# ColumbiaDVMM/ColumbiaImageSearch

Hardware: AMD Instinct MI355X
Metric: queries/sec @ recall@10 on 10M LOPQ index (higher is better)
Workload: dtype f64

## Files before the change

columbiaimagesearch_amd/_lib.py:

```python
import ctypes
import os
from ctypes import POINTER, c_char_p, c_double, c_float, c_int, c_int32, c_int64, c_uint8, c_uint16, c_uint32, c_void_p

import numpy as np

CIS_F32, CIS_F64 = 4, 8
CIS_OK, CIS_EINVAL, CIS_EHIP, CIS_ENOMEM, CIS_EUNSUPPORTED, CIS_ENODEVICE = 0, -1, -2, -3, -4, -5

_HERE = os.path.dirname(os.path.abspath(__file__))
LIB_PATH = os.environ.get("CIS_LIB_PATH") or os.path.join(_HERE, "lib", "libcis_hip.so")


class cis_hit(ctypes.Structure):
    _fields_ = [("dist", c_double), ("visit_rank", c_uint32), ("pos", c_uint32), ("id", c_int64),
                ("cell", c_int32), ("reserved", c_int32)]


HIT_DTYPE = np.dtype([("dist", "<f8"), ("visit_rank", "<u4"), ("pos", "<u4"), ("id", "<i8"),
                      ("cell", "<i4"), ("reserved", "<i4")])
assert HIT_DTYPE.itemsize == ctypes.sizeof(cis_hit) == 32


class HipError(RuntimeError):
    """A HIP runtime call inside libcis_hip.so failed (or no gfx950 device is visible)."""


_PROTOS = {
    "cis_version": (c_int, []),
    "cis_last_error": (c_char_p, []),
    "cis_alloc_stats": (c_int, [POINTER(c_int64), POINTER(c_int64)]),
    "cis_device_count": (c_int, []),
    "cis_set_device": (c_int, [c_int]),
    "cis_selftest": (c_int, [POINTER(c_int)]),
    "cis_model_create": (c_int, [POINTER(c_void_p), c_int, c_int, c_int, c_int, c_int, c_int, c_void_p, c_void_p,
                                 c_void_p, c_void_p, c_void_p, c_void_p, c_int, c_int]),
    "cis_model_destroy": (None, [c_void_p]),
    "cis_apply_pca": (c_int, [c_void_p, c_void_p, c_int, c_int64, c_void_p]),
    "cis_encode": (c_int, [c_void_p, c_void_p, c_int, c_int64, c_void_p, c_void_p]),
    "cis_encode_dev": (c_int, [c_void_p, c_void_p, c_int, c_int64, c_void_p, c_void_p, c_void_p]),
    "cis_predict_coarse": (c_int, [c_void_p, c_void_p, c_int, c_int64, c_void_p]),
    "cis_project": (c_int, [c_void_p, c_void_p, c_int, c_int64, c_void_p, c_void_p]),
    "cis_predict_fine": (c_int, [c_void_p, c_void_p, c_int, c_int64, c_void_p, c_void_p]),
    "cis_subquantizer_distances": (c_int, [c_void_p, c_void_p, c_int, c_int64, c_void_p, c_void_p]),
    "cis_reconstruct": (c_int, [c_void_p, c_void_p, c_void_p, c_int64, c_void_p]),
    "cis_predict_cluster": (c_int, [c_void_p, c_int, c_void_p, c_int, c_int64, c_int, c_int, c_void_p]),
    "cis_multisequence": (c_int, [c_void_p, c_int, c_void_p, c_void_p, c_int, c_int64, c_int, c_int, c_int, c_void_p, c_void_p,
                                  POINTER(c_int)]),
    "cis_index_create": (c_int, [POINTER(c_void_p), c_void_p]),
    "cis_index_destroy": (None, [c_void_p]),
    "cis_index_create_view": (c_int, [POINTER(c_void_p), c_void_p]),
    "cis_index_insert_counters": (c_int, [c_void_p, c_void_p]),
    "cis_index_set_shard": (c_int, [c_void_p, c_int, c_int, c_void_p]),
    "cis_index_cell_counts": (c_int, [c_void_p, c_void_p]),
    "cis_index_add_remote_counts": (c_int, [c_void_p, c_void_p]),
    "cis_index_add": (c_int, [c_void_p, c_void_p, c_void_p, c_void_p, c_int64, c_int, POINTER(c_int64)]),
    "cis_index_size": (c_int64, [c_void_p]),
    "cis_index_add_dev": (c_int, [c_void_p, c_void_p, c_void_p, c_void_p, c_int64, c_int, POINTER(c_int64), POINTER(c_int64),
                                  c_void_p, c_void_p]),
    "cis_l2_normalize_dev": (c_int, [c_void_p, c_int, c_int64, c_int, c_void_p]),
    "cis_index_cell_counts_dev": (c_int, [c_void_p, c_void_p, c_void_p]),
    "cis_index_add_remote_counts_dev": (c_int, [c_void_p, c_void_p, c_void_p]),
    "cis_index_route_pack_dev": (c_int, [c_void_p, c_void_p, c_void_p, c_void_p, c_int64, c_void_p, c_void_p, c_void_p]),
    "cis_index_add_records_dev": (c_int, [c_void_p, c_void_p, c_int64, c_int, POINTER(c_int64), POINTER(c_int64), c_void_p,
                                          c_void_p]),
    "cis_index_get_cell": (c_int, [c_void_p, c_int, c_int, c_int64, c_void_p, c_void_p, POINTER(c_int64)]),
    "cis_index_get_codes": (c_int, [c_void_p, c_void_p, c_void_p, c_int64, c_void_p]),
    "cis_index_search": (c_int, [c_void_p, c_void_p, c_int, c_int, c_int64, c_int, c_void_p, c_void_p, c_void_p,
                                 c_void_p, c_void_p, c_void_p]),
    "cis_index_search_async": (c_int, [c_void_p, c_void_p, c_int, c_int, c_int64, c_int, c_void_p, c_void_p, c_void_p,
                                       c_void_p, c_void_p, c_void_p]),
    "cis_index_search_wait": (c_int, [c_void_p]),
    "cis_host_alloc": (c_int, [POINTER(c_void_p), ctypes.c_size_t]),
    "cis_host_free": (None, [c_void_p]),
    "cis_index_search_dev": (c_int, [c_void_p, c_void_p, c_int, c_int, c_int64, c_int, c_void_p, c_void_p, c_void_p,
                                     c_void_p, c_void_p, c_void_p, c_void_p]),
    "cis_index_search_partial_dev": (c_int, [c_void_p, c_void_p, c_int, c_int, c_int64, c_int, c_void_p, c_void_p,
                                             c_void_p]),
    "cis_index_query_owners_dev": (c_int, [c_void_p, c_void_p, c_int, c_int, c_int64, c_void_p, c_void_p, c_void_p]),
    "cis_routed_merge_tables_dev": (c_int, [c_void_p, c_int, c_int, c_void_p, c_void_p, c_int, c_void_p, c_void_p, c_void_p]),
    "cis_route_queries_dev": (c_int, [c_void_p, c_int, c_int, c_void_p, c_int, c_int, c_void_p, c_void_p, c_void_p, c_void_p, c_void_p]),
    "cis_index_search_partial_packed_dev": (c_int, [c_void_p, c_void_p, c_int, c_int, c_int64, c_int, c_void_p, c_void_p,
                                                    c_void_p, c_void_p, c_void_p, c_void_p]),
    "cis_merge_hits_dev": (c_int, [c_void_p, c_int, c_int, c_int, c_void_p, c_void_p, c_void_p, c_void_p, c_void_p,
                                   c_void_p]),
    "cis_merge_packed_dev": (c_int, [c_void_p, c_int, c_int64, c_void_p, c_void_p, c_int, c_int, c_void_p, c_void_p,
                                     c_void_p, c_void_p, c_void_p, c_void_p]),
# ... 153 lines not shown
```

columbiaimagesearch_amd/csrc/lopq_search.hip:

```cpp
#include "lopq_batch.h"

template <typename CT>
__global__ __launch_bounds__(256) void k_tables(const CT* __restrict__ X , const CT* __restrict__ Cs,
                                                const double* __restrict__ Rt, const double* __restrict__ mus,
                                                const double* __restrict__ subs, const TabDesc* __restrict__ tabs,
                                                int V, int h, int w, int nf, int K, int D,
                                                double* __restrict__ T , PwProg prog_w,
                                                double* __restrict__ px_out ,
                                                const int* __restrict__ tab_order, int first) {
    extern __shared__ __attribute__((aligned(16))) char smem[];
    double* v = reinterpret_cast<double*>(smem);
    double* px = v + h;
    const int tab = tab_order ? tab_order[first + blockIdx.x] : first + (int)blockIdx.x;
    const TabDesc td = tabs[tab];
    const int s = td.split, c = td.cluster;
    const CT* x = X + (int64_t)td.q * D + s * h;
    const CT* Cc = Cs + ((int64_t)s * V + c) * h;
    const double* mu = mus + ((int64_t)s * V + c) * h;
    const double* R = Rt + ((int64_t)s * V + c) * h * h;
    for (int k = threadIdx.x; k < h; k += blockDim.x) {
        const CT res = x[k] - Cc[k];
        v[k] = (double)res - mu[k];
    }
    __syncthreads();
// ... 174 lines not shown
                for (int u = 0; u < CH; ++u) ra[u] = Ra[(int64_t)(s0 + u) * 4 * h];
#pragma unroll
                for (int u = 0; u < CH; ++u) rb[u] = vb[4 * (s0 + u)];
#pragma unroll
                for (int u = 0; u < CH; ++u) acc = __builtin_amdgcn_mfma_f64_16x16x4f64(ra[u], rb[u], acc, 0, 0, 0);
            }
            if (mine) {
                double* o = so + t * opitch + it * 16 + kq;
#pragma unroll
                for (int r = 0; r < 4; ++r) o[4 * r] = acc[r];
            }
        }
    }
    __syncthreads();
    for (int e = tid; e < nt * h; e += 256) {
        const int tt = e / h, i = e - tt * h;
        const double a = so[tt * opitch + i];
        px_out[(int64_t)s_tab[tt] * h + i] = a;
        if (px32_out) px32_out[(int64_t)s_tab[tt] * h + i] = (float)a;
    }
}

template <typename CT>
static void launch_tables(int64_t n_tabs, size_t tab_lds, hipStream_t st, const CT* X, const CT* Cs, const double* Rt,
                          const double* mus, const double* subs, const TabDesc* tabs, const int* tab_order, int V, int h, int w,
                          int nf, int K, int D, double* T, PwProg prog_w, double* px_out, const int64_t* d_totals = nullptr,
                          float* px32_out = nullptr) {
    constexpr int TB = 8;
    if (px_out && h <= 256 && h % 16 == 0 && !getenv("CIS_TABLES_UNGROUPED") && !getenv("CIS_TABLES_VALU")) {
        const size_t lds = (size_t)16 * (h + 4 + h + 2) * sizeof(double);
        if (h % 64 == 0)
            hipLaunchKernelGGL((k_tables_group_mfma<CT, 16>), dim3((unsigned)ceil_div(n_tabs, 16)), dim3(256), lds, st, X, Cs, Rt, mus, tabs,
                               tab_order, (int)n_tabs, V, h, D, px_out, d_totals, px32_out);
        else
            hipLaunchKernelGGL((k_tables_group_mfma<CT, 4>), dim3((unsigned)ceil_div(n_tabs, 16)), dim3(256), lds, st, X, Cs, Rt, mus, tabs,
                               tab_order, (int)n_tabs, V, h, D, px_out, d_totals, px32_out);
    } else if (px_out && h <= 256 && 256 / h >= 1 && !getenv("CIS_TABLES_UNGROUPED")) {
        const size_t lds = (size_t)(TB * h + TB * h) * sizeof(double);
        hipLaunchKernelGGL((k_tables_group<CT, TB>), dim3((unsigned)ceil_div(n_tabs, TB)), dim3(256), lds, st, X, Cs, Rt, mus, tabs,
                           tab_order, (int)n_tabs, V, h, D, px_out, d_totals, px32_out);
    } else {
        hipLaunchKernelGGL(k_tables<CT>, dim3((unsigned)n_tabs), dim3(256), tab_lds, st, X, Cs, Rt, mus, subs, tabs, V, h, w, nf, K, D, T,
                           prog_w, px_out, (const int*)nullptr, 0);
    }
}

template <int W, int TPB = 64>
__global__ __launch_bounds__(256) void k_tables_from_px(const double* __restrict__ px ,
                                                        TabDesc* __restrict__ tabs, int n_tabs,
                                                        const double* __restrict__ subs, int h, int nf, int K,
                                                        double* __restrict__ T ,
                                                        float* __restrict__ T32 ,
                                                        const int64_t* __restrict__ d_totals ) {
    __shared__ double sf[TPB][W];
    __shared__ int ssplit[TPB];
    const int j = blockIdx.y, z = blockIdx.z, k = threadIdx.x;
    const int t0 = blockIdx.x * TPB;
    if (d_totals) {
        n_tabs = (int)d_totals[1];
        if (t0 >= n_tabs) return;
    }
    const int nt = (n_tabs - t0 < TPB) ? (n_tabs - t0) : TPB;
    for (int e = threadIdx.x; e < nt * W; e += 256) {
        const int t = e / W, i = e - t * W;
        sf[t][i] = px[(int64_t)(t0 + t) * h + j * W + i];
    }
    if (threadIdx.x < nt) ssplit[threadIdx.x] = tabs[t0 + threadIdx.x].split;
    __syncthreads();
    const bool on = k < K;
    double sc[W];
    const double* src = subs + ((int64_t)(z * nf + j) * K + (on ? k : 0)) * W;
#pragma unroll
    for (int i = 0; i < W; ++i) sc[i] = src[i];
    for (int t = 0; t < nt; ++t) {
        if (ssplit[t] != z) continue;
        const double* f = sf[t];
        auto elem = [&](int i) -> double { const double df = f[i] - sc[i]; return df * df; };
        const double v = pw_leaf<double>(elem, 0, W);
        const float v32 = (float)v;
        if (on) {
            __builtin_nontemporal_store(v, &T[((int64_t)(t0 + t) * nf + j) * K + k]);
            if (T32) T32[((int64_t)(t0 + t) * nf + j) * K + k] = v32;
        }
        uint32_t b = on ? __float_as_uint(v32) : 0u, dummy = 0u;
        wave_minmax_step<1>(dummy, b); wave_minmax_step<2>(dummy, b); wave_minmax_step<4>(dummy, b);
        wave_minmax_step<8>(dummy, b); wave_minmax_step<16>(dummy, b); wave_minmax_step<32>(dummy, b);
        if ((threadIdx.x & 63) == 0) atomicMax(reinterpret_cast<unsigned int*>(&tabs[t0 + t].pad), b);
    }
}

__global__ void k_tables_f32(const double* __restrict__ T, int64_t n, int nf, int K, float* __restrict__ T32, TabDesc* __restrict__ tabs) {
    const int64_t e = (int64_t)blockIdx.x * blockDim.x + threadIdx.x;
    if (e >= n) return;
    const float v = (float)T[e];
    T32[e] = v;
    atomicMax(reinterpret_cast<unsigned int*>(&tabs[e / ((int64_t)nf * K)].pad), __float_as_uint(v));
}

template <int N, int NT, bool PAY>
__device__ __forceinline__ void block_bitonic(uint64_t* ka, uint64_t* kb, int64_t* pay) {
    for (int k = 2; k <= N; k <<= 1) {
        for (int j = k >> 1; j > 0; j >>= 1) {
            for (int t = threadIdx.x; t < N / 2; t += NT) {
                const int i = ((t / j) * 2 * j) + (t % j);
                const int p = i + j;
                const bool asc = ((i & k) == 0);
                const uint64_t a0 = ka[i], b0 = kb[i], a1 = ka[p], b1 = kb[p];
                const bool gt = (a0 > a1) || (a0 == a1 && b0 > b1);
                if (gt == asc) {
                    ka[i] = a1; kb[i] = b1; ka[p] = a0; kb[p] = b0;
                    if (PAY) { const int64_t x = pay[i]; pay[i] = pay[p]; pay[p] = x; }
                }
            }
            __syncthreads();
        }
    }
}

template <int M>
__device__ __forceinline__ double adc_one(const uint8_t* __restrict__ codes, int64_t p, const double* __restrict__ T, int K) {
    double d;
    if constexpr (M == 4) {
        const uint32_t c = *reinterpret_cast<const uint32_t*>(codes + p * 4);
        d = T[c & 255];
        d = d + T[K + ((c >> 8) & 255)];
        d = d + T[2 * K + ((c >> 16) & 255)];
        d = d + T[3 * K + (c >> 24)];
    } else if constexpr (M == 8) {
        const uint2 c = *reinterpret_cast<const uint2*>(codes + p * 8);
        d = T[c.x & 255];
        d = d + T[K + ((c.x >> 8) & 255)];
        d = d + T[2 * K + ((c.x >> 16) & 255)];
        d = d + T[3 * K + (c.x >> 24)];
        d = d + T[4 * K + (c.y & 255)];
        d = d + T[5 * K + ((c.y >> 8) & 255)];
        d = d + T[6 * K + ((c.y >> 16) & 255)];
        d = d + T[7 * K + (c.y >> 24)];
    } else if constexpr (M == 16) {
        const uint4 c = *reinterpret_cast<const uint4*>(codes + p * 16);
        const uint32_t cw[4] = {c.x, c.y, c.z, c.w};
// ... 956 lines not shown
            const uint32_t rank = (uint32_t)(kb[x] >> 32), pos = (uint32_t)kb[x];
            int64_t src = -1;
            int cell = -1;
#pragma unroll
            for (int li = 3; li >= 0; --li) {
                const uint32_t rel = pos - l_pos0[li];
                if (l_rank[li] == rank && rel < l_len[li]) {
                    src = l_start[li] + rel;
                    cell = l_cell[li];
                }
            }
            for (int li = 4; li < n_lists && src < 0; ++li) {
                const WorkItem it = items[first + li];
                const uint32_t rel = pos - (uint32_t)it.pos0;
                if ((uint32_t)it.rank == rank && rel < (uint32_t)it.len) {
                    src = it.start + rel;
                    cell = it.cell;
                }
            }
            if (src >= 0) {
                hh.dist = __longlong_as_double((long long)ka[x]);
                hh.visit_rank = rank;
                hh.pos = pos;
                hh.id = ids[src];
                hh.cell = cell;
            }
        }
        if (out_hits) out_hits[o + x] = hh;
        if (out_ids) {
            out_ids[o + x] = hh.id;
            out_dists[o + x] = (x < nv) ? hh.dist : __longlong_as_double(0x7ff8000000000000LL);
        }
        if (out_cells) out_cells[o + x] = hh.cell;
        if (out_pos) out_pos[o + x] = hh.pos;
    }
    if (lane == 0 && out_n) out_n[q] = nv;
}

__global__ void k_copy_visited(const PlanOut* __restrict__ plan, int nq, int32_t* __restrict__ visited) {
    const int q = blockIdx.x * blockDim.x + threadIdx.x;
    if (q < nq) visited[q] = plan[q].visited;
}


extern "C" int cis_index_set_profiling(cis_index* ix, int enable) {
    CIS_REQUIRE(ix != nullptr, "index is NULL");
    ix->profiling = enable < 0 ? 0 : (enable > 2 ? 2 : enable);
    return CIS_OK;
}

template <int LJ>
__device__ int selftest_xor(uint32_t v) { return lane_xor<LJ>(v) != (uint32_t)__shfl_xor((int)v, LJ) ? 1 : 0; }

template <int NR>
__device__ int selftest_sort(uint32_t seed) {
    const int lane = threadIdx.x & 63;
    uint32_t k[NR];
#pragma unroll
    for (int r = 0; r < NR; ++r) {
        uint32_t x = seed ^ (uint32_t)(lane * NR + r) * 2654435761u;
        x ^= x >> 15; x *= 2246822519u; x ^= x >> 13;
        k[r] = x % 1000u;
    }
    uint32_t mine[NR];
#pragma unroll
    for (int r = 0; r < NR; ++r) mine[r] = k[r];
    wave_bitonic_sort<NR>(k);
    int bad = 0;
#pragma unroll
    for (int r = 0; r + 1 < NR; ++r) bad += k[r] > k[r + 1];
    const uint32_t nxt = (uint32_t)__shfl_down((int)k[0], 1);
    if (lane < 63) bad += k[NR - 1] > nxt;
    uint32_t s0 = 0, s1 = 0, x0 = 0, x1 = 0;
#pragma unroll
    for (int r = 0; r < NR; ++r) { s0 += mine[r]; s1 += k[r]; x0 ^= mine[r] * 40503u; x1 ^= k[r] * 40503u; }
    for (int o = 32; o > 0; o >>= 1) {
        s0 += (uint32_t)__shfl_xor((int)s0, o); s1 += (uint32_t)__shfl_xor((int)s1, o);
        x0 ^= (uint32_t)__shfl_xor((int)x0, o); x1 ^= (uint32_t)__shfl_xor((int)x1, o);
    }
    bad += (s0 != s1) + (x0 != x1);
    return bad;
}

static __device__ uint32_t selftest_hash(uint32_t x) {
    x *= 2654435761u; x ^= x >> 15; x *= 2246822519u; x ^= x >> 13;
    return x;
}

template <int NR>
__device__ int selftest_cut(int c, uint32_t seed) {
    __shared__ uint32_t s_hi[NR * 64], s_lo[NR * 64], s_out[NR * 64];
    const int lane = threadIdx.x & 63;
    const int cnt = NR * 64 - 8 - (int)seed * 5 - c;
    const int L = c == 0 ? cnt + 3 : (c == 1 ? cnt : (c == 7 ? cnt / 3 : (c == 2 ? cnt * 2 / 3 : cnt / 2 - (int)seed)));
    uint32_t hi[NR], lo[NR], mn = 0xffffffffu, mx = 0u;
    bool keep[NR];
#pragma unroll
    for (int r = 0; r < NR; ++r) {
        const uint32_t e = (uint32_t)(r * 64 + lane), h = selftest_hash(seed * 4099u + e), h2 = selftest_hash(h + 1u);
        const uint32_t distinct = (e * 167u + seed) % 1021u;
        keep[r] = (int)e < cnt;
        hi[r] = c == 2 ? distinct : (c == 3 || c == 4 ? h % 3u : (c == 5 ? h % 2u : (c == 6 ? 5u : h % 1000u)));
        lo[r] = c == 3 ? h2 % 50u : (c == 4 ? hi[r] * 7u + 1u : (c == 5 ? distinct : (c == 6 ? 9u : h2)));
        s_hi[e] = hi[r]; s_lo[e] = lo[r];
        mn = (keep[r] && hi[r] < mn) ? hi[r] : mn;
        mx = (keep[r] && hi[r] > mx) ? hi[r] : mx;
// ... 13 lines not shown
        for (int e = 0; e < cnt; ++e) {
            int c_e = 0;
            for (int f = 0; f < cnt; ++f) c_e += s_hi[f] <= s_hi[e];
            if (c_e >= n && s_hi[e] < nth) nth = s_hi[e];
            c_ref += s_hi[e] <= v;
            k_min = s_hi[e] < k_min ? s_hi[e] : k_min;
            k_max = s_hi[e] > k_max ? s_hi[e] : k_max;
            if (pred(s_lo[e])) { bad += s_out[j] != s_lo[e]; ++j; }
        }
        bad += (mn != k_min) + (mx != k_max) + (c_v != c_ref) + (c_ref < n) + (c_ref > n + W && v != nth) + (j != n_kept);
        bad += (c == 3 || c == 6) && v != nth;
        bad += (cnt >= L ? v_guard != v : v_guard != mx);
    }
    wave_lds_sync();
    uint32_t vhiL = 0u, dup_pos = 0xffffffffu;
    uint64_t boundL = 0ull;
    wave_exact_cut<NR>(hi, lo, keep, [&](int r) { return 7u * (uint32_t)(r * 64 + lane) + 3u; }, mn, mx, cnt, L, vhiL, boundL, dup_pos);
#pragma unroll
    for (int r = 0; r < NR; ++r) s_out[r * 64 + lane] = keep[r] ? 1u : 0u;
    wave_lds_sync();
    if (lane == 0) {
        int kth = -1;
        for (int e = 0; e < NR * 64; ++e) {
            int before = 0;
            for (int f = 0; f < cnt; ++f)
                before += s_hi[f] < s_hi[e] || (s_hi[f] == s_hi[e] && (s_lo[f] < s_lo[e] || (s_lo[f] == s_lo[e] && f < e)));
            bad += s_out[e] != ((e < cnt && before < L) ? 1u : 0u);
            if (e < cnt && before == L - 1) kth = e;
        }
        uint32_t dup_ref = 0xffffffffu;
        if (kth >= 0) {
            int c_less = 0, g = 0, first = -1;
            for (int e = cnt - 1; e >= 0; --e) {
                c_less += s_hi[e] < s_hi[kth];
                g += s_hi[e] == s_hi[kth];
                if (s_hi[e] == s_hi[kth] && s_lo[e] == s_lo[kth]) first = e;
            }
            if (L - c_less < g) dup_ref = 7u * (uint32_t)first + 3u;
        }
        bad += (kth >= 0) != (cnt >= L);
        bad += vhiL != (kth >= 0 ? s_hi[kth] : mx);
        bad += boundL != (kth >= 0 ? hi_to_bound(s_hi[kth]) : 0x7ff0000000000000ull);
        bad += dup_pos != dup_ref;
        bad += (c == 4 || c == 6) && dup_ref == 0xffffffffu;
    }
    return bad;
}

__global__ void k_selftest(int* __restrict__ errors) {
    const uint32_t v = (uint32_t)threadIdx.x * 7919u + blockIdx.x * 104729u + 17u;
    int bad = selftest_xor<1>(v) + selftest_xor<2>(v) + selftest_xor<4>(v) + selftest_xor<8>(v) + selftest_xor<16>(v) +
              selftest_xor<32>(v);
    bad += selftest_sort<4>(blockIdx.x * 977u + 1u) + selftest_sort<8>(blockIdx.x * 31u + 5u);
    bad += selftest_cut<4>(blockIdx.x & 7, blockIdx.x >> 3) + selftest_cut<8>(blockIdx.x & 7, blockIdx.x >> 3);
    if (bad) atomicAdd(errors, bad);
}

#ifdef CIS_SCAN_COUNTERS
extern "C" int cis_debug_counters(unsigned long long* out, int reset) {
    CIS_CHECK_HIP(hipMemcpyFromSymbol(out, HIP_SYMBOL(g_scan_ctr), 16 * sizeof(unsigned long long)));
    if (reset) {
        unsigned long long z[16] = {0};
        CIS_CHECK_HIP(hipMemcpyToSymbol(HIP_SYMBOL(g_scan_ctr), z, sizeof(z)));
    }
    return CIS_OK;
}
#endif

extern "C" int cis_selftest(int* n_errors) {
    CIS_REQUIRE(n_errors != nullptr, "NULL argument");
    CIS_TRY(cis_lazy_init());
    int* d = nullptr;
    CIS_CHECK_HIP(hipMalloc((void**)&d, sizeof(int)));
    CIS_CHECK_HIP(hipMemset(d, 0, sizeof(int)));
    hipLaunchKernelGGL(k_selftest, dim3(64), dim3(64), 0, nullptr, d);
    CIS_CHECK_HIP(hipMemcpy(n_errors, d, sizeof(int), hipMemcpyDeviceToHost));
    (void)hipFree(d);
    return CIS_OK;
}

extern "C" int cis_index_set_scan_mode(cis_index* ix, int mode) {
    CIS_REQUIRE(ix != nullptr && mode >= 0 && mode <= 7, "bad scan mode");
    if (mode == 7) mode = 5;
    ix->force_stream = (mode == 6);
    ix->force_exact_scan = (mode == 1);
    ix->force_prefilter_scan = (mode >= 2 && mode <= 5);
    ix->force_scan2 = (mode == 2);
    ix->force_scan3 = (mode == 3 || mode == 4 || mode == 5);
    ix->force_two_pass = mode == 3 ? 0 : (mode == 4 ? 1 : (mode == 5 ? 2 : -1));
    return CIS_OK;
}

extern "C" int cis_index_read_profile(cis_index* ix, double ms[5], int64_t* launches) {
    CIS_REQUIRE(ix != nullptr && ms != nullptr, "NULL argument");
    for (auto& r : ix->prof) {
        hipEvent_t last = r.ev[4] ? r.ev[4] : r.ev[3];
        if (last) CIS_CHECK_HIP(hipEventSynchronize(last));
        for (int i = 0; i < 4; ++i) {
            if (!r.ev[i] || !r.ev[i + 1]) continue;
            float t = 0.f;
            CIS_CHECK_HIP(hipEventElapsedTime(&t, r.ev[i], r.ev[i + 1]));
            ix->prof_ms[i] += t;
        }
        if (r.has_scan && r.ev[5] && r.ev[3]) {
            float t = 0.f;
            CIS_CHECK_HIP(hipEventElapsedTime(&t, r.ev[5], r.ev[3]));
// ... 1373 lines not shown
                (ix->force_stream || b.d_tot != nullptr || b.n_cand_all / (nq > 0 ? nq : 1) >= r->stream_min);
    if (!r->stream) {
        const int64_t S_ = r->fast ? r->geom.S : L;
        double need = (double)b.n_items * S_ * (r->fast ? sizeof(uint64_t) : sizeof(cis_hit)) + (double)b.n_tabs * nf * K * sizeof(double);
        if (r->big) {
            const SelectPlan sp_ = select_plan(L, nq, b.n_cand_all);
            need = (sp_.select ? 8.0 * (double)b.n_cand_all + (sp_.sort_lds ? 16.0 : 32.0) * (double)nq * (double)sp_.stride : 32.0 * (double)b.n_cand_all) +
                   (r->direct ? (double)b.n_tabs * h * sizeof(double) : (double)b.n_tabs * nf * K * sizeof(double));
        }
        const double budget = (getenv("CIS_WORKSPACE_GB") ? atof(getenv("CIS_WORKSPACE_GB")) : 24.0) * 1.0e9;
        if (need > budget && nq > 1) {
            ix->retry_fraction = 0.9 * budget / need;
            return CIS_RETRY_SMALLER;
        }
    }
    if (!b.d_tot) {
        ix->stats[0] += b.n_cand_all;
        ix->stats[1] += b.n_items;
        ix->stats[2] += b.n_tabs;
    }
    r->geom3 = scan3_geom(M, K, L, b.n_items > 0 ? b.n_cand_all / b.n_items : 0, ix->force_two_pass);
    r->S = r->fast ? (r->use3 ? r->geom3.S : r->geom.S) : L;
    static const bool no_t32 = getenv("CIS_NO_T32") != nullptr && atoi(getenv("CIS_NO_T32")) != 0;
    r->drop_t32 = no_t32 && !r->direct && r->split_tables;
    return CIS_OK;
}

static int reserve_batch(Batch& b, const Route& r) {
    cis_index* ix = b.ix;
    cis_model* m = ix->m;
    const int K = m->K, h = m->h, nf = m->nf;
    const int64_t n_items = b.n_items, n_tabs = b.n_tabs;
    CIS_TRY(ix->w_items.reserve((size_t)(n_items + 1) * sizeof(WorkItem)));
    CIS_TRY(ix->w_tabs.reserve((size_t)(n_tabs + 1) * sizeof(TabDesc)));
    CIS_TRY(ix->w_T.reserve(r.direct ? 256 : (size_t)(n_tabs + 1) * nf * K * sizeof(double)));
    if (!r.big && !r.stream) CIS_TRY(ix->w_hits.reserve((size_t)(n_items + 1) * r.S * (r.fast ? sizeof(uint64_t) : sizeof(cis_hit))));
    CIS_TRY(ix->w_hitn.reserve((size_t)(n_items + 1) * 2 * sizeof(int)));
    if (r.use3) CIS_TRY(ix->w_slack.reserve((size_t)(n_items + 1) * 2 * sizeof(float)));
    b.items = ix->w_items.as<WorkItem>();
    b.tabs = ix->w_tabs.as<TabDesc>();
    CIS_TRY(ix->w_tord.reserve((size_t)(n_tabs + 1) * sizeof(int)));
    b.tab_order = ix->w_tord.as<int>();
    b.T = ix->w_T.as<double>();
    if (!r.drop_t32) CIS_TRY(ix->w_T32.reserve(r.direct ? (size_t)(n_tabs + 1) * h * sizeof(float) : (size_t)(n_tabs + 1) * nf * K * sizeof(float)));
    b.T32 = r.drop_t32 ? nullptr : ix->w_T32.as<float>();
    b.px_buf = nullptr;
    if (r.split_tables) {
        CIS_TRY(ix->w_px.reserve((size_t)(n_tabs + 1) * h * sizeof(double)));
        b.px_buf = ix->w_px.as<double>();
    }
    return CIS_OK;
}

static void finish_tables(const Batch& b, const Route& r) {
    cis_model* m = b.ix->m;
    hipStream_t st = b.st;
    const int K = m->K, h = m->h, nf = m->nf;
    const int64_t n_tabs = b.n_tabs;
    double *T = b.T, *px_buf = b.px_buf;
    float* T32 = b.T32;
    TabDesc* tabs = b.tabs;
    const int64_t* d_tot = b.d_tot;
    if (r.direct) {
    } else if (r.split_tables && n_tabs > 0) {
        const bool few = n_tabs <= 1024;
        dim3 g((unsigned)ceil_div(n_tabs, few ? 8 : 64), (unsigned)nf, 2);
#define CIS_TFP(WW)                                                                                                                                      \
        if (few) hipLaunchKernelGGL((k_tables_from_px<WW, 8>), g, dim3(256), 0, st, px_buf, tabs, (int)n_tabs, m->d_subs, h, nf, K, T, T32, d_tot);      \
        else hipLaunchKernelGGL((k_tables_from_px<WW, 64>), g, dim3(256), 0, st, px_buf, tabs, (int)n_tabs, m->d_subs, h, nf, K, T, T32, d_tot)
        switch (m->w) {
            case 4: CIS_TFP(4); break;
            case 8: CIS_TFP(8); break;
            case 16: CIS_TFP(16); break;
            default: CIS_TFP(32); break;
        }
#undef CIS_TFP
    } else if (r.fast && n_tabs > 0) {
        const int64_t ne = n_tabs * nf * K;
        hipLaunchKernelGGL(k_tables_f32, dim3((unsigned)ceil_div(ne, 256)), dim3(256), 0, st, T, ne, nf, K, T32, tabs);
    }
}

static int search_batch(cis_index* ix, const void* dQ, int q_dtype, int nq, int64_t quota, int L, const SearchOut& out, hipStream_t st);

static int run_stream(Batch& b, const Route& r) {
    cis_index* ix = b.ix;
    hipStream_t st = b.st;
    const int K = ix->m->K, M = ix->m->M, nq = b.nq, L = b.L;
    const int64_t n_items = b.n_items, n_cand_all = b.n_cand_all;
    const SearchOut& out = b.out;
    CIS_TRY(mark(b, 2));
    const uint8_t* codes = ix->codes_ptr();
    const int64_t* ids = ix->ids_ptr();
    const bool shared_cells = b.quota >= ix->n_total / 2;
    const int G = (nq >= 3 && shared_cells && stream_max_group() >= 4) ? 4 : (nq >= 2 ? 2 : 1);
    const int cap = STREAM_CAP, B = STREAM_B;
    const SelectPlan sp = select_plan(L, nq, (int64_t)nq * cap);
    CIS_REQUIRE(sp.sort_lds, "streaming route: limit above the LDS-ranked range");
    int64_t CH = ceil_div(ix->max_cell > 0 ? ix->max_cell : 1, (int64_t)r.seg_max);
    CH = CH < 1 ? 1 : (CH > 16 ? 16 : CH);
    Slots sl;
    CIS_TRY(build_slots(b, G > 1 ? SLOTS_SORTED : SLOTS_NONE, G, CH, r.seg_max, &sl));
    const int64_t max_slots = sl.max_slots;
    {
        const size_t need = (size_t)nq * B * sizeof(uint32_t);
        if (need > ix->w_bmin.cap) {
            CIS_TRY(ix->w_bmin.reserve(need > (size_t)16 * B * sizeof(uint32_t) ? need : (size_t)16 * B * sizeof(uint32_t)));
            CIS_CHECK_HIP(hipMemsetAsync(ix->w_bmin.p, 0xff, ix->w_bmin.cap, st));
        }
    }
    const size_t n_i64 = (size_t)(n_items + 1) + (size_t)3 * (nq + 2) + (size_t)(max_slots + 2) + (size_t)(max_slots + 1) * ((stream_slot_bytes() + 7) / 8);
    const size_t bytes = n_i64 * 8 + (size_t)(nq + 2) * 4 * 4 + (size_t)nq * cap * 4 + (size_t)nq * cap * 8 + (size_t)2 * nq * sp.stride * 8 + 1024;
    CIS_TRY(ix->w_hits.reserve(bytes));
    int64_t* cand_start = ix->w_hits.as<int64_t>();
    int64_t* seg = cand_start + (n_items + 1);
    unsigned long long* qmin = reinterpret_cast<unsigned long long*>(seg + (nq + 2));
    unsigned long long* qmax = qmin + (nq + 2);
    int64_t* rowoff = reinterpret_cast<int64_t*>(qmax + (nq + 2));
    void* sdesc = rowoff + (max_slots + 2);
    uint64_t* skeys = reinterpret_cast<uint64_t*>(rowoff + (max_slots + 2) + (size_t)(max_slots + 1) * ((stream_slot_bytes() + 7) / 8));
    uint64_t* sel_keys = skeys + (size_t)nq * cap;
    uint64_t* sel_vals = sel_keys + (size_t)nq * sp.stride;
    uint32_t* surv = reinterpret_cast<uint32_t*>(sel_vals + (size_t)nq * sp.stride);
    uint32_t* bmin = ix->w_bmin.as<uint32_t>();
    int* cnt = reinterpret_cast<int*>(surv + (size_t)nq * cap);
    int* nsel = cnt + (nq + 2);
    float* tau = reinterpret_cast<float*>(nsel + (nq + 2));
    int* status = reinterpret_cast<int*>(tau + (nq + 2));
    const CandArgs c{st, b.items, n_items, b.item_off, cand_start, seg, qmin, qmax, nq, codes, K};
    StreamArgs s{};
    s.M = M; s.G = G; s.L = L;
    s.slots = sl.slots; s.n_slots = sl.n_slots; s.rowoff = rowoff; s.desc = sdesc;
    s.T = b.T; s.T32 = b.T32; s.tau = tau; s.bmin = bmin; s.B = B;
// ... 410 lines not shown
```

columbiaimagesearch_amd/csrc/scan_common.h:

```cpp
#pragma once
#include <type_traits>

#include "lopq_model.h"

struct WorkItem {
    int q;
    int rank;
    int tab0, tab1;
    int64_t start;
    int len;
    int pos0;
    int cell;
    int pad;
};

struct TabDesc {
    int q, split, cluster, pad;
};

struct PlanOut {
    int visited, n_items, ntab0, ntab1;
    int64_t ncand;
};

// ... 26 lines not shown
    const int lane = threadIdx.x & 63;
    if constexpr (J < NR) {
#pragma unroll
        for (int r = 0; r < NR; ++r) {
            if ((r & J) == 0) {
                const bool asc = (((lane * NR + r) & KK) == 0);
                const uint32_t a = k[r], b = k[r | J];
                const uint32_t lo = a < b ? a : b, hi = a < b ? b : a;
                k[r] = asc ? lo : hi;
                k[r | J] = asc ? hi : lo;
            }
        }
    } else {
        constexpr int LJ = J / NR;
        const bool lower = ((lane & LJ) == 0);
        const bool asc = (((lane * NR) & KK) == 0);
#pragma unroll
        for (int r = 0; r < NR; ++r) {
            const uint32_t o = lane_xor<LJ>(k[r]);
            const uint32_t mn = k[r] < o ? k[r] : o, mx = k[r] < o ? o : k[r];
            k[r] = (lower == asc) ? mn : mx;
        }
    }
}

template <int NR, int KK, int J>
__device__ __forceinline__ void bitonic_merge(uint32_t (&k)[NR]) {
    bitonic_step<NR, KK, J>(k);
    if constexpr (J > 1) bitonic_merge<NR, KK, J / 2>(k);
}

template <int NR, int KK>
__device__ __forceinline__ void bitonic_levels(uint32_t (&k)[NR]) {
    if constexpr (KK > 2) bitonic_levels<NR, KK / 2>(k);
    bitonic_merge<NR, KK, KK / 2>(k);
}

template <int NR>
__device__ __forceinline__ void wave_bitonic_sort(uint32_t (&k)[NR]) {
    bitonic_levels<NR, NR * 64>(k);
}

template <int LJ>
__device__ __forceinline__ void wave_minmax_step(uint32_t& mn, uint32_t& mx) {
    const uint32_t a = lane_xor<LJ>(mn), b = lane_xor<LJ>(mx);
    mn = a < mn ? a : mn;
    mx = b > mx ? b : mx;
}
static __device__ __forceinline__ void wave_minmax_all(uint32_t& mn, uint32_t& mx) {
    wave_minmax_step<1>(mn, mx); wave_minmax_step<2>(mn, mx); wave_minmax_step<4>(mn, mx);
    wave_minmax_step<8>(mn, mx); wave_minmax_step<16>(mn, mx); wave_minmax_step<32>(mn, mx);
    mn = (uint32_t)__builtin_amdgcn_readfirstlane((int)mn);
    mx = (uint32_t)__builtin_amdgcn_readfirstlane((int)mx);
}

template <int NR>
__device__ __forceinline__ uint32_t wave_kth_bisect(const uint32_t (&key)[NR], const bool (&valid)[NR], uint32_t lo,
                                                    uint32_t hi, int target) {
    while (lo < hi) {
        const uint32_t p = lo + ((hi - lo) >> 1);
        int c = 0;
#pragma unroll
        for (int r = 0; r < NR; ++r) c += __popcll(__ballot(valid[r] && key[r] <= p));
        if (c >= target) hi = p;
        else lo = p + 1;
    }
    return lo;
}

template <int NR>
__device__ __forceinline__ int wave_count_le(const bool (&keep)[NR], const uint32_t (&key)[NR], uint32_t p) {
    int c = 0;
#pragma unroll
    for (int r = 0; r < NR; ++r) c += __popcll(__ballot(keep[r] && key[r] <= p));
    return c;
}

template <int NR>
__device__ __forceinline__ uint32_t wave_bisect_window(const bool (&keep)[NR], const uint32_t (&key)[NR], uint32_t lo, uint32_t hi,
                                                       int n, int W) {
    while (lo < hi) {
        const uint32_t p = lo + ((hi - lo) >> 1);
        const int c = wave_count_le<NR>(keep, key, p);
        if (c >= n) {
            hi = p;
            if (c <= n + W) break;
        } else {
            lo = p + 1;
        }
    }
    return hi;
}

template <int NR, typename P, typename S>
__device__ __forceinline__ int wave_stable_keep(P&& pred, S&& store) {
    int n = 0;
#pragma unroll
    for (int r = 0; r < NR; ++r) {
        const bool kp = pred(r);
        const unsigned long long m = __ballot(kp);
        const int idx = n + __builtin_amdgcn_mbcnt_hi((unsigned)(m >> 32), __builtin_amdgcn_mbcnt_lo((unsigned)m, 0));
        if (kp) store(r, idx);
        n += __popcll(m);
    }
    __builtin_amdgcn_fence(__ATOMIC_RELEASE, "wavefront");
    __builtin_amdgcn_wave_barrier();
// ... 415 lines not shown
```

include/cis_hip.h:

```cpp
#ifndef CIS_HIP_H
#define CIS_HIP_H

#include <stddef.h>
#include <stdint.h>

#ifdef __cplusplus
extern "C" {
#endif

#define CIS_F32 4
#define CIS_F64 8

#define CIS_OK 0
#define CIS_EINVAL -1
#define CIS_EHIP -2
#define CIS_ENOMEM -3
#define CIS_EUNSUPPORTED -4
#define CIS_ENODEVICE -5

typedef struct cis_model cis_model;
typedef struct cis_index cis_index;
typedef struct cis_cnn cis_cnn;

typedef struct cis_hit {
    double dist;
    uint32_t visit_rank;
    uint32_t pos;
    int64_t id;
    int32_t cell;
    int32_t reserved;
} cis_hit;

int cis_version(void);
const char* cis_last_error(void);
int cis_alloc_stats(int64_t* n_allocs, int64_t* n_bytes);
int cis_device_count(void);
int cis_set_device(int device);
int cis_selftest(int* n_errors);

int cis_model_create(cis_model** out, int D_in, int D, int V, int M, int K, int coarse_dtype,
                     const void* Cs, const double* Rs, const double* mus, const double* subs,
                     const double* pca_P, const double* pca_mu, int pca_mu_dtype, int renorm);
void cis_model_destroy(cis_model* m);

int cis_apply_pca(cis_model* m, const void* X, int x_dtype, int64_t n, float* out);

int cis_encode(cis_model* m, const void* X, int x_dtype, int64_t n, uint16_t* coarse, uint8_t* fine);
int cis_encode_dev(cis_model* m, const void* dX, int x_dtype, int64_t n, uint16_t* d_coarse,
                   uint8_t* d_fine, void* stream);

int cis_predict_coarse(cis_model* m, const void* X, int x_dtype, int64_t n, uint16_t* coarse);
int cis_project(cis_model* m, const void* X, int x_dtype, int64_t n, const uint16_t* coarse, double* out);
int cis_predict_fine(cis_model* m, const void* X, int x_dtype, int64_t n, const uint16_t* coarse, uint8_t* fine);
int cis_subquantizer_distances(cis_model* m, const void* X, int x_dtype, int64_t n,
                               const uint16_t* coarse, double* tables);
int cis_reconstruct(cis_model* m, const uint16_t* coarse, const uint8_t* fine, int64_t n, double* out);

int cis_predict_cluster(const void* X, int x_dtype, const void* C, int c_dtype, int64_t n, int ncent, int d,
                        uint32_t* out);

int cis_multisequence(const void* X, int x_dtype, const void* C0, const void* C1, int c_dtype, int64_t n, int V,
                      int h, int max_cells, int32_t* cells, double* dists, int* dist_dtype);

int cis_index_create(cis_index** out, cis_model* m);
void cis_index_destroy(cis_index* ix);
int cis_index_create_view(cis_index** out, cis_index* base);

int cis_index_set_shard(cis_index* ix, int rank, int world, const int32_t* owner );
int cis_index_insert_counters(cis_index* ix, int64_t counters[2]);

int cis_index_cell_counts(cis_index* ix, int64_t* counts);
int cis_index_add_remote_counts(cis_index* ix, const int64_t* delta);
int cis_index_cell_counts_dev(cis_index* ix, int64_t* d_counts, void* stream);
int cis_index_add_remote_counts_dev(cis_index* ix, const int64_t* d_delta, void* stream);
int cis_index_route_pack_dev(cis_index* ix, const int64_t* d_ids, const uint16_t* d_coarse, const uint8_t* d_fine,
                             int64_t n, uint8_t* d_records, int64_t* d_counts, void* stream);
int cis_index_add_records_dev(cis_index* ix, const uint8_t* d_records, int64_t n, int dedup, int64_t* n_added,
                              int64_t* n_invalid, int64_t* d_cell_delta, void* stream);

int cis_index_add(cis_index* ix, const int64_t* ids, const uint16_t* coarse, const uint8_t* fine,
                  int64_t n, int dedup, int64_t* n_added);
int cis_index_add_dev(cis_index* ix, const int64_t* d_ids, const uint16_t* d_coarse, const uint8_t* d_fine, int64_t n,
                      int dedup, int64_t* n_added, int64_t* n_invalid, int64_t* d_cell_delta ,
                      void* stream);
int cis_l2_normalize_dev(void* d_x, int dtype, int64_t n, int d, void* stream);
int64_t cis_index_size(cis_index* ix);
int cis_index_get_cell(cis_index* ix, int c0, int c1, int64_t cap, int64_t* ids, uint8_t* fine, int64_t* n);

int cis_index_search(cis_index* ix, const void* Q, int q_dtype, int nq, int64_t quota, int limit,
                     int64_t* ids, double* dists, int32_t* n_found, int32_t* visited,
                     int32_t* cells, uint32_t* pos);
// ... 88 lines not shown
```

Measured before the change: 25.07 million.

## Persist k_tables_from_px blocks over table ranges with ballot-driven pairwise evaluation

The tables-from-projection kernel becomes grid-stride style: each block walks a contiguous range of tables in chunks, loading codeword centroids once and prefetching px rows into registers before staging them in LDS. Tables whose split differs are skipped through a wave ballot, and two tables are processed per iteration. Their row maxima are reduced with a transposed 16-lane max that feeds LDS atomics instead of one global atomic per wave per table. The launch caps the grid at a resident-occupancy count for wide subvectors, and a debug entry point plus a selftest are added. The aim is less redundant centroid loading, wasted iterations and global atomics, at the cost of more complex indexing and less parallelism when there are few tables.

```diff
diff --git a/columbiaimagesearch_amd/_lib.py b/columbiaimagesearch_amd/_lib.py
--- a/columbiaimagesearch_amd/_lib.py
+++ b/columbiaimagesearch_amd/_lib.py
@@ -32,6 +32,7 @@
     "cis_device_count": (c_int, []),
     "cis_set_device": (c_int, [c_int]),
     "cis_selftest": (c_int, [POINTER(c_int)]),
+    "cis_debug_tables_from_px": (c_int, [c_void_p, c_void_p, c_void_p, c_int64, c_void_p, c_void_p, c_void_p]),
     "cis_model_create": (c_int, [POINTER(c_void_p), c_int, c_int, c_int, c_int, c_int, c_int, c_void_p, c_void_p,
                                  c_void_p, c_void_p, c_void_p, c_void_p, c_int, c_int]),
     "cis_model_destroy": (None, [c_void_p]),
diff --git a/columbiaimagesearch_amd/csrc/lopq_search.hip b/columbiaimagesearch_amd/csrc/lopq_search.hip
--- a/columbiaimagesearch_amd/csrc/lopq_search.hip
+++ b/columbiaimagesearch_amd/csrc/lopq_search.hip
@@ -250,40 +250,69 @@
                                                         double* __restrict__ T ,
                                                         float* __restrict__ T32 ,
                                                         const int64_t* __restrict__ d_totals ) {
-    __shared__ double sf[TPB][W];
-    __shared__ int ssplit[TPB];
-    const int j = blockIdx.y, z = blockIdx.z, k = threadIdx.x;
-    const int t0 = blockIdx.x * TPB;
-    if (d_totals) {
-        n_tabs = (int)d_totals[1];
-        if (t0 >= n_tabs) return;
-    }
-    const int nt = (n_tabs - t0 < TPB) ? (n_tabs - t0) : TPB;
-    for (int e = threadIdx.x; e < nt * W; e += 256) {
-        const int t = e / W, i = e - t * W;
-        sf[t][i] = px[(int64_t)(t0 + t) * h + j * W + i];
-    }
-    if (threadIdx.x < nt) ssplit[threadIdx.x] = tabs[t0 + threadIdx.x].split;
-    __syncthreads();
+    static_assert(TPB <= 64, "a chunk's tables are one ballot");
+    constexpr int NS = (TPB * W + 255) / 256;
+    __shared__ __attribute__((aligned(16))) double sf[TPB][W];
+    __shared__ uint32_t smax[TPB];
+    const int j = blockIdx.y, z = blockIdx.z, k = threadIdx.x, lane = threadIdx.x & 63;
+    if (d_totals) n_tabs = (int)d_totals[1];
+    int per = (n_tabs + (int)gridDim.x - 1) / (int)gridDim.x;
+    per = per < TPB ? TPB : per;
+    const int r0 = blockIdx.x * per, r1 = r0 + per < n_tabs ? r0 + per : n_tabs;
+    if (r0 >= n_tabs) return;
+    const int n_chunks = (r1 - r0 + TPB - 1) / TPB, chunk = (r1 - r0 + n_chunks - 1) / n_chunks;
     const bool on = k < K;
     double sc[W];
     const double* src = subs + ((int64_t)(z * nf + j) * K + (on ? k : 0)) * W;
 #pragma unroll
     for (int i = 0; i < W; ++i) sc[i] = src[i];
-    for (int t = 0; t < nt; ++t) {
-        if (ssplit[t] != z) continue;
-        const double* f = sf[t];
-        auto elem = [&](int i) -> double { const double df = f[i] - sc[i]; return df * df; };
-        const double v = pw_leaf<double>(elem, 0, W);
-        const float v32 = (float)v;
-        if (on) {
-            __builtin_nontemporal_store(v, &T[((int64_t)(t0 + t) * nf + j) * K + k]);
-            if (T32) T32[((int64_t)(t0 + t) * nf + j) * K + k] = v32;
-        }
-        uint32_t b = on ? __float_as_uint(v32) : 0u, dummy = 0u;
-        wave_minmax_step<1>(dummy, b); wave_minmax_step<2>(dummy, b); wave_minmax_step<4>(dummy, b);
-        wave_minmax_step<8>(dummy, b); wave_minmax_step<16>(dummy, b); wave_minmax_step<32>(dummy, b);
-        if ((threadIdx.x & 63) == 0) atomicMax(reinterpret_cast<unsigned int*>(&tabs[t0 + t].pad), b);
+    if (k < TPB) smax[k] = 0u;
+    for (int t0 = r0; t0 < r1; t0 += chunk) {
+        const int nt = r1 - t0 < chunk ? r1 - t0 : chunk;
+        double sv[NS];
+#pragma unroll
+        for (int u = 0; u < NS; ++u) {
+            const int e = k + 256 * u, t = e / W, i = e - t * W;
+            sv[u] = px[(int64_t)(t0 + (t < nt ? t : nt - 1)) * h + j * W + i];
+        }
+        const int split = lane < nt ? tabs[t0 + lane].split : -1;
+#pragma unroll
+        for (int u = 0; u < NS; ++u)
+            if (k + 256 * u < TPB * W) (&sf[0][0])[k + 256 * u] = sv[u];
+        __syncthreads();
+        const uint64_t mine = __ballot(split == z);
+        for (uint64_t left = mine; left != 0;) {
+            int t[2];
+            t[0] = __builtin_ctzll(left);
+            left &= left - 1;
+            const bool live[2] = {true, left != 0};
+            t[1] = live[1] ? __builtin_ctzll(left) : t[0];
+            left &= left - 1;
+            double v[2];
+#pragma unroll
+            for (int u = 0; u < 2; ++u) {
+                const double* f = sf[t[u]];
+                auto elem = [&](int i) -> double { const double df = f[i] - sc[i]; return df * df; };
+                v[u] = pw_leaf<double>(elem, 0, W);
+            }
+            uint32_t b[2];
+#pragma unroll
+            for (int u = 0; u < 2; ++u) {
+                const float v32 = (float)v[u];
+                if (on && live[u]) {
+                    __builtin_nontemporal_store(v[u], &T[((int64_t)(t0 + t[u]) * nf + j) * K + k]);
+                    if (T32) T32[((int64_t)(t0 + t[u]) * nf + j) * K + k] = v32;
+                }
+                b[u] = on ? __float_as_uint(v32) : 0u;
+            }
+            const uint32_t m = row_max2_transposed(b[0], b[1]);
+            if ((lane & 14) == 0) atomicMax(&smax[(lane & 1) ? t[1] : t[0]], m);
+        }
+        __syncthreads();
+        if (k < nt) {
+            if ((mine >> k) & 1) atomicMax(reinterpret_cast<unsigned int*>(&tabs[t0 + k].pad), smax[k]);
+            smax[k] = 0u;
+        }
     }
 }
 
@@ -1346,6 +1375,24 @@
 template <int LJ>
 __device__ int selftest_xor(uint32_t v) { return lane_xor<LJ>(v) != (uint32_t)__shfl_xor((int)v, LJ) ? 1 : 0; }
 
+__device__ int selftest_row_max2(uint32_t seed) {
+    const int lane = threadIdx.x & 63;
+    uint32_t b[2], want[2];
+#pragma unroll
+    for (int u = 0; u < 2; ++u) {
+        uint32_t x = seed ^ (uint32_t)(lane * 2 + u) * 2654435761u;
+        x ^= x >> 15; x *= 2246822519u; x ^= x >> 13;
+        b[u] = (seed & 1u) ? x % 7u : x;
+        want[u] = b[u];
+#pragma unroll
+        for (int d = 1; d < 16; d <<= 1) {
+            const uint32_t o = (uint32_t)__shfl_xor((int)want[u], d);
+            want[u] = o > want[u] ? o : want[u];
+        }
+    }
+    return row_max2_transposed(b[0], b[1]) != ((lane & 1) ? want[1] : want[0]) ? 1 : 0;
+}
+
 template <int NR>
 __device__ int selftest_sort(uint32_t seed) {
     const int lane = threadIdx.x & 63;
@@ -1465,6 +1512,7 @@
     int bad = selftest_xor<1>(v) + selftest_xor<2>(v) + selftest_xor<4>(v) + selftest_xor<8>(v) + selftest_xor<16>(v) +
               selftest_xor<32>(v);
     bad += selftest_sort<4>(blockIdx.x * 977u + 1u) + selftest_sort<8>(blockIdx.x * 31u + 5u);
+    bad += selftest_row_max2(blockIdx.x * 7919u + 3u);
     bad += selftest_cut<4>(blockIdx.x & 7, blockIdx.x >> 3) + selftest_cut<8>(blockIdx.x & 7, blockIdx.x >> 3);
     if (bad) atomicAdd(errors, bad);
 }
@@ -2944,33 +2992,78 @@
     return CIS_OK;
 }
 
+static int tables_from_px_blocks_per_cu(int w) { return w <= 8 ? 8 : (w <= 16 ? 4 : 2); }
+
+static void launch_tables_from_px(const cis_model* m, hipStream_t st, const double* px, TabDesc* tabs, int64_t n_tabs, double* T,
+                                  float* T32, const int64_t* d_tot) {
+    const int K = m->K, h = m->h, nf = m->nf;
+    const bool few = n_tabs <= 1024;
+    const int64_t want = ceil_div(n_tabs, few ? 8 : 64), resident = 256 * tables_from_px_blocks_per_cu(m->w) / (2 * nf);
+    const bool one_round = m->w >= 16 && want > resident && resident >= 1;
+    dim3 g((unsigned)(one_round ? resident : want), (unsigned)nf, 2);
+#define CIS_TFP(WW)                                                                                                                              \
+    if (few) hipLaunchKernelGGL((k_tables_from_px<WW, 8>), g, dim3(256), 0, st, px, tabs, (int)n_tabs, m->d_subs, h, nf, K, T, T32, d_tot);      \
+    else hipLaunchKernelGGL((k_tables_from_px<WW, 64>), g, dim3(256), 0, st, px, tabs, (int)n_tabs, m->d_subs, h, nf, K, T, T32, d_tot)
+    switch (m->w) {
+        case 4: CIS_TFP(4); break;
+        case 8: CIS_TFP(8); break;
+        case 16: CIS_TFP(16); break;
+        default: CIS_TFP(32); break;
+    }
+#undef CIS_TFP
+}
+
 static void finish_tables(const Batch& b, const Route& r) {
     cis_model* m = b.ix->m;
     hipStream_t st = b.st;
-    const int K = m->K, h = m->h, nf = m->nf;
+    const int K = m->K, nf = m->nf;
     const int64_t n_tabs = b.n_tabs;
-    double *T = b.T, *px_buf = b.px_buf;
+    double* T = b.T;
     float* T32 = b.T32;
     TabDesc* tabs = b.tabs;
-    const int64_t* d_tot = b.d_tot;
     if (r.direct) {
     } else if (r.split_tables && n_tabs > 0) {
-        const bool few = n_tabs <= 1024;
-        dim3 g((unsigned)ceil_div(n_tabs, few ? 8 : 64), (unsigned)nf, 2);
-#define CIS_TFP(WW)                                                                                                                                      \
-        if (few) hipLaunchKernelGGL((k_tables_from_px<WW, 8>), g, dim3(256), 0, st, px_buf, tabs, (int)n_tabs, m->d_subs, h, nf, K, T, T32, d_tot);      \
-        else hipLaunchKernelGGL((k_tables_from_px<WW, 64>), g, dim3(256), 0, st, px_buf, tabs, (int)n_tabs, m->d_subs, h, nf, K, T, T32, d_tot)
-        switch (m->w) {
-            case 4: CIS_TFP(4); break;
-            case 8: CIS_TFP(8); break;
-            case 16: CIS_TFP(16); break;
-            default: CIS_TFP(32); break;
-        }
-#undef CIS_TFP
+        launch_tables_from_px(m, st, b.px_buf, tabs, n_tabs, T, T32, b.d_tot);
     } else if (r.fast && n_tabs > 0) {
         const int64_t ne = n_tabs * nf * K;
         hipLaunchKernelGGL(k_tables_f32, dim3((unsigned)ceil_div(ne, 256)), dim3(256), 0, st, T, ne, nf, K, T32, tabs);
     }
+}
+
+extern "C" int cis_debug_tables_from_px(cis_model* m, const double* px, const int32_t* split, int64_t n_tabs, double* T, float* T32,
+                                        int32_t* pad) {
+    CIS_REQUIRE(m && px && split && T && T32 && pad, "NULL argument");
+    CIS_REQUIRE(n_tabs > 0 && n_tabs <= (1 << 20), "n_tabs must be in 1 .. 2^20");
+    CIS_REQUIRE(m->K <= 256 && (m->w == 4 || m->w == 8 || m->w == 16 || m->w == 32), "k_tables_from_px serves K <= 256 and w in 4, 8, 16, 32");
+    std::vector<TabDesc> td((size_t)n_tabs);
+    for (int64_t t = 0; t < n_tabs; ++t) {
+        CIS_REQUIRE(split[t] == 0 || split[t] == 1, "split must be 0 or 1");
+        td[t] = TabDesc{0, split[t], 0, 0};
+    }
+    CIS_TRY(cis_lazy_init());
+    const size_t ne = (size_t)n_tabs * m->nf * m->K;
+    DevBuf d_px, d_td, d_T, d_T32;
+    const auto run = [&]() -> int {
+        CIS_TRY(d_px.reserve((size_t)n_tabs * m->h * sizeof(double)));
+        CIS_TRY(d_td.reserve((size_t)n_tabs * sizeof(TabDesc)));
+        CIS_TRY(d_T.reserve(ne * sizeof(double)));
+        CIS_TRY(d_T32.reserve(ne * sizeof(float)));
+        CIS_CHECK_HIP(hipMemcpy(d_px.p, px, (size_t)n_tabs * m->h * sizeof(double), hipMemcpyHostToDevice));
+        CIS_CHECK_HIP(hipMemcpy(d_td.p, td.data(), (size_t)n_tabs * sizeof(TabDesc), hipMemcpyHostToDevice));
+        CIS_CHECK_HIP(hipMemset(d_T.p, 0xff, ne * sizeof(double)));
+        CIS_CHECK_HIP(hipMemset(d_T32.p, 0xff, ne * sizeof(float)));
+        launch_tables_from_px(m, nullptr, d_px.as<double>(), d_td.as<TabDesc>(), n_tabs, d_T.as<double>(), d_T32.as<float>(), nullptr);
+        CIS_CHECK_HIP(hipGetLastError());
+        CIS_CHECK_HIP(hipMemcpy(T, d_T.p, ne * sizeof(double), hipMemcpyDeviceToHost));
+        CIS_CHECK_HIP(hipMemcpy(T32, d_T32.p, ne * sizeof(float), hipMemcpyDeviceToHost));
+        CIS_CHECK_HIP(hipMemcpy(td.data(), d_td.p, (size_t)n_tabs * sizeof(TabDesc), hipMemcpyDeviceToHost));
+        return CIS_OK;
+    };
+    const int rc = run();
+    d_px.release(); d_td.release(); d_T.release(); d_T32.release();
+    CIS_TRY(rc);
+    for (int64_t t = 0; t < n_tabs; ++t) pad[t] = td[t].pad;
+    return CIS_OK;
 }
 
 static int search_batch(cis_index* ix, const void* dQ, int q_dtype, int nq, int64_t quota, int L, const SearchOut& out, hipStream_t st);
diff --git a/columbiaimagesearch_amd/csrc/scan_common.h b/columbiaimagesearch_amd/csrc/scan_common.h
--- a/columbiaimagesearch_amd/csrc/scan_common.h
+++ b/columbiaimagesearch_amd/csrc/scan_common.h
@@ -102,6 +102,18 @@
     wave_minmax_step<8>(mn, mx); wave_minmax_step<16>(mn, mx); wave_minmax_step<32>(mn, mx);
     mn = (uint32_t)__builtin_amdgcn_readfirstlane((int)mn);
     mx = (uint32_t)__builtin_amdgcn_readfirstlane((int)mx);
+}
+
+static __device__ __forceinline__ uint32_t row_max2_transposed(uint32_t b0, uint32_t b1) {
+    const bool odd = (threadIdx.x & 1) != 0;
+    const uint32_t r = lane_xor<1>(odd ? b0 : b1), k = odd ? b1 : b0;
+    uint32_t m = r > k ? r : k;
+    const uint32_t m2 = lane_xor<2>(m);
+    m = m2 > m ? m2 : m;
+    const uint32_t m4 = lane_xor<4>(m);
+    m = m4 > m ? m4 : m;
+    const uint32_t m8 = lane_xor<8>(m);
+    return m8 > m ? m8 : m;
 }
 
 template <int NR>
diff --git a/include/cis_hip.h b/include/cis_hip.h
--- a/include/cis_hip.h
+++ b/include/cis_hip.h
@@ -37,6 +37,8 @@
 int cis_device_count(void);
 int cis_set_device(int device);
 int cis_selftest(int* n_errors);
+int cis_debug_tables_from_px(cis_model* m, const double* px, const int32_t* split, int64_t n_tabs, double* T, float* T32,
+                             int32_t* pad);
 
 int cis_model_create(cis_model** out, int D_in, int D, int V, int M, int K, int coarse_dtype,
                      const void* Cs, const double* Rs, const double* mus, const double* subs,
```

After: 25.06 million (median of 3 runs). No clear change (-0.1%).
